# jiahansu/GPUAR

Measured on AMD Instinct MI355X. Metric: encode+decode GB/s, higher is better.
Workload: dtype u16

## Files before the change

### gpuar_amd/csrc/gpuar_kernels.hip

```cpp
#include <hip/hip_runtime.h>
#include <mutex>
#include <stdint.h>
#include <stdio.h>
#include <stdlib.h>
#include <string.h>

#include "gpuar_hip.h"

#include "lane_codec.h"
#include "crc32.h"

namespace gpuar {

__constant__ RecipTable g_recip = RecipTable();
struct MulTable {
    uint32_t m[kPacket + 64];
    constexpr MulTable() : m{} {
        const RecipTable r = RecipTable();
        for (uint32_t i = 0; i < kPacket + 64; ++i) m[i] = r.r[i < kPacket ? i : kPacket - 1u].mul;
    }
};
__device__ const MulTable g_mul = MulTable();
__constant__ DecodeConstTable g_decode = DecodeConstTable();
__device__ uint32_t g_status = 0;
// ... 19 lines not shown
        const uint32_t other = __shfl_xor(v, off);
        v = other > v ? other : v;
    }
    return __builtin_amdgcn_readfirstlane(v);
}

constexpr uint32_t kPhase = 8;
constexpr int kPrioTop = 3, kPrioCoder = 0, kPrioLow = 2;

constexpr uint32_t kRingSlots = 3;
struct alignas(16) EncodeLds {
    uint8_t tree[kTreeRows * kLanes * 2];
    uint32_t sums[kRingSlots][kPhase][kLanes];
    uint32_t bytes[2][kPhase / 4][kLanes];
};
__device__ __forceinline__ uint32_t next_slot(uint32_t slot) { return slot == kRingSlots - 1u ? 0u : slot + 1u; }

__device__ __forceinline__ size_t xcd_contiguous_group(uint32_t block, uint32_t grid) {
    const uint32_t per_xcd = grid >> 3;
    return static_cast<size_t>(block & 7u) * per_xcd + (block >> 3);
}

__device__ __forceinline__ void lds_barrier() {
    asm volatile("s_waitcnt lgkmcnt(0)\n\ts_barrier" ::: "memory");
}

__device__ __forceinline__ uint4 load16_guarded(const uint8_t *p, size_t avail) {
    if (avail >= 16) return *reinterpret_cast<const uint4 *>(p);
    uint32_t w[4] = {0, 0, 0, 0};
    for (size_t b = 0; b < avail; ++b) w[b >> 2] |= static_cast<uint32_t>(p[b]) << (8u * (b & 3u));
    return make_uint4(w[0], w[1], w[2], w[3]);
}

__device__ __forceinline__ uint32_t byte_tag(uint32_t word, uint32_t kByte) {
    uint32_t t;
    const uint32_t seven = 7u;
    if (kByte == 0) asm("v_lshlrev_b32_sdwa %0, %1, %2 dst_sel:DWORD dst_unused:UNUSED_PAD src0_sel:DWORD src1_sel:BYTE_0" : "=v"(t) : "v"(seven), "v"(word));
    if (kByte == 1) asm("v_lshlrev_b32_sdwa %0, %1, %2 dst_sel:DWORD dst_unused:UNUSED_PAD src0_sel:DWORD src1_sel:BYTE_1" : "=v"(t) : "v"(seven), "v"(word));
    if (kByte == 2) asm("v_lshlrev_b32_sdwa %0, %1, %2 dst_sel:DWORD dst_unused:UNUSED_PAD src0_sel:DWORD src1_sel:BYTE_2" : "=v"(t) : "v"(seven), "v"(word));
    if (kByte == 3) asm("v_lshlrev_b32_sdwa %0, %1, %2 dst_sel:DWORD dst_unused:UNUSED_PAD src0_sel:DWORD src1_sel:BYTE_3" : "=v"(t) : "v"(seven), "v"(word));
    return t;
}

template <bool kBatch = false>
__device__ __forceinline__ void run_top(EncodeLds &lds, const uint8_t *in, uint32_t lane, uint32_t len,
                                        uint32_t len_min, uint32_t n_phases, uint32_t whole_max = 0) {
    constexpr uint32_t kChunkPhases = 8;
    constexpr uint32_t kChunk = kChunkPhases * kPhase;
    constexpr uint32_t kPieces = kChunk / 16u;
    TopModeler<7> model;
    uint32_t k = 0, slot = 0;
    {
        const uint32_t first = len ? load16_guarded(in, len).x & 0xFFu : 0u;
        model.open(lds.tree, 2u * lane_column(lane), first);
    }
    const uint32_t full_chunks = len_min / kChunk;
    if (full_chunks) {
        const uint4 *src = reinterpret_cast<const uint4 *>(in);
        auto fetch = [&](uint32_t chunk, uint4 (&into)[kPieces]) {
#pragma unroll
            for (uint32_t t = 0; t < kPieces; ++t) {
                const uint32_t at = chunk * kChunk + 16u * t;
                if (at + 16u <= len) into[t] = src[kPieces * chunk + t];
                else if (at < len) into[t] = load16_guarded(in + at, len - at);
                else into[t] = make_uint4(0, 0, 0, 0);
            }
        };
        uint4 c[kPieces], n[kPieces], nn[kPieces];
        fetch(0, c);
        fetch(1, n);
#pragma unroll
        for (uint32_t t = 0; t < kPieces; ++t) nn[t] = make_uint4(0, 0, 0, 0);
        for (uint32_t q = 0; q < full_chunks; ++q) {
            if (q & 1u) {
                fetch(q + 1u, n);
                fetch(q + 2u, nn);
            }
            uint32_t w[kChunk / 4u + 1u];
#pragma unroll
            for (uint32_t t = 0; t < kPieces; ++t) w[4 * t] = c[t].x, w[4 * t + 1] = c[t].y, w[4 * t + 2] = c[t].z, w[4 * t + 3] = c[t].w;
            w[kChunk / 4u] = n[0].x;
#pragma unroll
            for (uint32_t ph = 0; ph < kChunkPhases; ++ph) {
                uint32_t *out = &lds.sums[slot][0][lane];
                lds.bytes[ph & 1u][0][lane] = w[2 * ph];
                lds.bytes[ph & 1u][1][lane] = w[2 * ph + 1];
#pragma unroll
                for (uint32_t j = 0; j < kPhase; ++j) {
                    const uint32_t i = ph * kPhase + j;
                    const uint32_t xn_tag = byte_tag(w[(i + 1) >> 2], (i + 1) & 3u);
                    out[j * kLanes] = model.step_tag(model.next_tag, 256u + q * kChunk + i, xn_tag);
                }
                slot = next_slot(slot);
                lds_barrier();
            }
#pragma unroll
            for (uint32_t t = 0; t < kPieces; ++t) c[t] = n[t], n[t] = nn[t];
        }
        k = kChunkPhases * full_chunks;
    }
    uint4 cur = make_uint4(0, 0, 0, 0), nxt = cur;
    if (k * kPhase < len) cur = load16_guarded(in + k * kPhase, len - k * kPhase);
    if (k * kPhase + 16u < len) nxt = load16_guarded(in + k * kPhase + 16u, len - (k * kPhase + 16u));
    if constexpr (kBatch) {
        const uint32_t whole = len / kPhase;
        for (; k < whole_max; ++k) {
            const uint32_t base = k * kPhase;
// ... 22 lines not shown
            const uint32_t own = whole * kPhase, part = len - own;
            const uint4 v = part ? load16_guarded(in + own, part) : make_uint4(0, 0, 0, 0);
            lds.bytes[k & 1u][0][lane] = v.x;
            lds.bytes[k & 1u][1][lane] = v.y;
            uint32_t *out = &lds.sums[slot][0][lane];
            uint64_t w = (static_cast<uint64_t>(v.y) << 32) | v.x;
#pragma unroll 1
            for (uint32_t j = 0; j < part; ++j) {
                const uint32_t x = static_cast<uint32_t>(w) & 0xFFu;
                w >>= 8;
                out[j * kLanes] = model.step(x, 256u + own + j, static_cast<uint32_t>(w) & 0xFFu);
            }
            slot = next_slot(slot);
            lds_barrier();
            ++k;
        }
        for (; k < n_phases + 2u; ++k) lds_barrier();
        return;
    }
    for (; k < n_phases + 2u; ++k) {
        if (k < n_phases) {
            const uint32_t base = k * kPhase;
            const bool odd = (k & 1u) != 0u;
            const uint32_t words[3] = {odd ? cur.z : cur.x, odd ? cur.w : cur.y, odd ? nxt.x : cur.z};
            if (odd) {
                cur = nxt;
                const uint32_t ahead = base + kPhase + 16u;
                if (ahead < len) nxt = load16_guarded(in + ahead, len - ahead);
                else nxt = make_uint4(0, 0, 0, 0);
            }
            uint32_t *out = &lds.sums[slot][0][lane];
            lds.bytes[k & 1u][0][lane] = words[0];
            lds.bytes[k & 1u][1][lane] = words[1];
#pragma unroll
            for (uint32_t q = 0; q < 2; ++q) {
                uint32_t w = words[q], w_next = words[q + 1];
#pragma unroll 1
                for (uint32_t b = 0; b < 4; ++b) {
                    const uint32_t i = base + 4u * q + b;
                    const uint32_t x = w & 0xFFu;
                    w = (w >> 8) | (w_next << 24);
                    w_next >>= 8;
                    if (i < len) *out = model.step(x, 256u + i, w & 0xFFu);
                    out += kLanes;
                }
            }
            slot = next_slot(slot);
        }
        lds_barrier();
    }
}

__device__ __forceinline__ void run_low(EncodeLds &lds, uint32_t lane, uint32_t len, uint32_t len_min, uint32_t n_phases) {
    LowModeler<7> model;
    model.open(lds.tree, 2u * lane_column(lane), 0u);
    lds_barrier();
    uint32_t slot = 0, k = 0;
    const uint32_t whole_phases = len_min / kPhase < n_phases ? len_min / kPhase : n_phases;
    for (; k < whole_phases; ++k) {
        const uint32_t base = k * kPhase;
        uint32_t *io = &lds.sums[slot][0][lane];
        {
            uint32_t part[kPhase], tag[kPhase];
            const uint32_t bytes[2] = {lds.bytes[k & 1u][0][lane], lds.bytes[k & 1u][1][lane]};
#pragma unroll
            for (uint32_t j = 0; j < kPhase; ++j) part[j] = io[j * kLanes], tag[j] = byte_tag(bytes[j >> 2], j & 3u);
            model.prime_tag(tag[0]);
#pragma unroll
            for (uint32_t j = 0; j < kPhase; ++j) {
                if (j + 1u < kPhase) io[j * kLanes] = model.step_tag(tag[j], 256u + base + j, tag[j + 1u], part[j]);
                else io[j * kLanes] = model.step_last_tag(tag[j], 256u + base + j, part[j]);
            }
        }
        slot = next_slot(slot);
        lds_barrier();
    }
    for (; k < n_phases; ++k) {
        const uint32_t base = k * kPhase;
        uint32_t *io = &lds.sums[slot][0][lane];
        const uint32_t bytes[2] = {lds.bytes[k & 1u][0][lane], lds.bytes[k & 1u][1][lane]};
        {
#pragma unroll 1
            for (uint32_t j = 0; j < kPhase; ++j) {
                const uint32_t i = base + j;
                if (i < len) {
                    const uint32_t t = model.tree.tag((bytes[j >> 2] >> (8u * (j & 3u))) & 0xFFu);
                    model.prime_tag(t);
                    io[j * kLanes] = model.step_last_tag(t, 256u + i, io[j * kLanes]);
                }
            }
        }
        slot = next_slot(slot);
        lds_barrier();
    }
    lds_barrier();
}

template <typename Coder>
__device__ __forceinline__ void coder_open(Coder &coder, uint8_t *dst, size_t group, uint32_t lane) {
    __builtin_amdgcn_s_setprio(kPrioCoder);
    coder.open(dst + group * (kLanes * kSlot), lane * kSlot);
    lds_barrier();
    lds_barrier();
}

template <typename Lane>
__device__ __forceinline__ void finish_lane(Lane &coder, bool live, uint32_t len, uint32_t *status) {
    if (live) {
// ... 7 lines not shown
encode_kernel(const uint8_t *__restrict__ src, size_t size, uint8_t *__restrict__ dst, uint32_t n_packets, uint32_t *__restrict__ status) {
    __shared__ EncodeLds lds;

    const size_t group = xcd_contiguous_group(blockIdx.x, gridDim.x);
    if (group * kLanes >= n_packets) return;
    const uint32_t lane = threadIdx.x & 63u;
    const uint32_t wave = __builtin_amdgcn_readfirstlane(threadIdx.x >> 6);
    const uint32_t hw = __builtin_amdgcn_s_getreg(4 | (0 << 6) | (31 << 11));
    const uint32_t simd = (hw >> 4) & 3u;
    uint32_t *hello = &lds.sums[0][0][0];
    if (lane == 0) hello[wave] = simd;
    if (threadIdx.x == 0) {
        const uint32_t xcc = __builtin_amdgcn_s_getreg(20 | (0 << 6) | (3 << 11));
        hello[4] = atomicAdd(&g_cu_ticket[((xcc & 7u) << 8) | ((hw >> 8) & 0xFFu)], 1u);
    }
    __syncthreads();
    const uint32_t seen = (1u << hello[0]) | (1u << hello[1]) | (1u << hello[2]) | (1u << hello[3]);
    const uint32_t by_simd = (simd - hello[4] - 1u) & 3u;
    const uint32_t role = __builtin_amdgcn_readfirstlane(seen == 0xFu ? by_simd : wave);
    __syncthreads();
    const size_t packet = group * kLanes + lane;
    const bool live = packet < n_packets;
    const size_t start = packet * kPacket;
    const uint32_t len = live ? static_cast<uint32_t>(size - start < kPacket ? size - start : kPacket) : 0u;
    const uint32_t len_max = wave_max(len);
    const uint32_t len_min = wave_max(~len) ^ 0xFFFFFFFFu;
    const uint32_t n_phases = (len_max + kPhase - 1) / kPhase;
    const uint8_t *in = src + (live ? start : 0);

    if (role == 0) {
        __builtin_amdgcn_s_setprio(kPrioTop);
        run_top(lds, in, lane, len, len_min, n_phases);
    } else if (role == 1) {
        __builtin_amdgcn_s_setprio(kPrioLow);
        run_low(lds, lane, len, len_min, n_phases);
    } else if (role == 3) {
        uint32_t *courier = reinterpret_cast<uint32_t *>(lds.tree + 255u * 128u);
        const uint32_t *table = reinterpret_cast<const uint32_t *>(g_recip.r);
        const uint32_t lane16 = lane & 15u;
        clock_sample(0u, group, lane, 0u);
        uint32_t carried = table[lane16];
        for (uint32_t k = 0; k < n_phases + 2u; ++k) {
            if (lane < 16u) courier[((k + 1u) & 1u) * 16u + lane16] = carried;
            const uint32_t next_phase = k < n_phases ? k : 0u;
            carried = table[next_phase * 16u + lane16];
            lds_barrier();
        }
        clock_sample(0u, group, lane, 1u);
    } else {
        CarryCoderLane coder;
        coder_open(coder, dst, group, lane);
        uint32_t slot = 0, k = 0;
        const uint32_t whole_phases = len_min / kPhase < n_phases ? len_min / kPhase : n_phases;
        for (; k < whole_phases; ++k) {
            const uint32_t *in_ring = &lds.sums[slot][0][lane];
            {
                uint32_t cums[kPhase];
#pragma unroll
                for (uint32_t j = 0; j < kPhase; ++j) cums[j] = in_ring[j * kLanes];
                Recip rc[kPhase];
                {
                    const uint4 *slot = reinterpret_cast<const uint4 *>(lds.tree + 255u * 128u + (k & 1u) * 64u);
#pragma unroll
                    for (uint32_t q = 0; q < 4; ++q) {
                        const uint4 v = slot[q];
                        rc[2 * q] = {v.x, v.y}, rc[2 * q + 1] = {v.z, v.w};
                    }
                }
                CarryCoderLane::Ahead next = coder.ahead(cums[0], rc[0]);
#pragma unroll
                for (uint32_t j = 0; j < kPhase; ++j) {
                    const CarryCoderLane::Narrowed now = coder.narrow(next);
                    if (j + 1u < kPhase) next = coder.ahead(cums[j + 1u], rc[j + 1u]);
                    coder.settle(now);
                }
            }
            slot = next_slot(slot);
            lds_barrier();
        }
        for (; k < n_phases; ++k) {
            const uint32_t base = k * kPhase;
            const uint32_t *in_ring = &lds.sums[slot][0][lane];
            {
#pragma unroll 1
                for (uint32_t j = 0; j < kPhase; ++j) {
                    const uint32_t i = base + j;
                    if (i >= len_max) break;
                    const Recip r = g_recip.r[i];
                    if (i < len) coder.step(in_ring[j * kLanes], r);
                }
            }
            slot = next_slot(slot);
            lds_barrier();
        }
        if (live) {
            bool overflowed;
            coder.finish(len, overflowed);
            if (overflowed) atomicOr(status, GPUAR_STATUS_SLOT_OVERFLOW);
        }
    }
}

__device__ __forceinline__ void batch_low(EncodeLds &lds, uint32_t lane, uint32_t len, uint32_t len_min, uint32_t n_phases, uint32_t whole_max) {
    LowModeler<7> model;
    model.open(lds.tree, 2u * lane_column(lane), 0u);
    lds_barrier();
    uint32_t slot = 0, k = 0;
    auto whole_phase = [&](uint32_t k) __attribute__((always_inline)) {
        const uint32_t base = k * kPhase;
        uint32_t *io = &lds.sums[slot][0][lane];
        uint32_t part[kPhase], tag[kPhase];
        const uint32_t bytes[2] = {lds.bytes[k & 1u][0][lane], lds.bytes[k & 1u][1][lane]};
#pragma unroll
        for (uint32_t j = 0; j < kPhase; ++j) part[j] = io[j * kLanes], tag[j] = byte_tag(bytes[j >> 2], j & 3u);
        model.prime_tag(tag[0]);
#pragma unroll
        for (uint32_t j = 0; j < kPhase; ++j) {
            if (j + 1u < kPhase) io[j * kLanes] = model.step_tag(tag[j], 256u + base + j, tag[j + 1u], part[j]);
            else io[j * kLanes] = model.step_last_tag(tag[j], 256u + base + j, part[j]);
        }
    };
    const uint32_t whole_min = len_min / kPhase;
    for (; k < whole_min; ++k) {
        whole_phase(k);
        slot = next_slot(slot);
        lds_barrier();
    }
    const uint32_t whole = len / kPhase;
// ... 1682 lines not shown
```

### gpuar_amd/csrc/lane_codec.h

```cpp
#ifndef GPUAR_LANE_CODEC_H
#define GPUAR_LANE_CODEC_H

#include <stdint.h>
#include <string.h>

#include "gpuar_hip.h"
#if defined(__HIP_DEVICE_COMPILE__) || defined(__HIPCC__)
#define GPUAR_LANE __device__ __forceinline__
#define GPUAR_CLZ32(x) static_cast<uint32_t>(__clz(static_cast<int>(x)))
#define GPUAR_CLZ32_NZ(x) static_cast<uint32_t>(__builtin_clz(x))
#define GPUAR_MULHI(a, b) __umulhi((a), (b))
#define GPUAR_MUL24(a, b) __umul24((a), (b))
#define GPUAR_AGREE_COUNT(kff, a, h, span) ([](uint32_t &k_, uint32_t a_, uint32_t h_, uint32_t &s_) { uint32_t e_; asm("v_xor_b32_sdwa %0, %3, %4 dst_sel:WORD_1 dst_unused:UNUSED_PRESERVE src0_sel:DWORD src1_sel:DWORD\n\tv_bfi_b32 %1, %3, %4, -1\n\tv_ffbh_u32 %2, %0" : "+v"(k_), "=&v"(s_), "=&v"(e_) : "v"(a_), "v"(h_)); return e_; }((kff), (a), (h), (span)))
#define GPUAR_BFM(w, off) ([](uint32_t w_, uint32_t o_) { uint32_t r_; asm("v_bfm_b32 %0, %1, %2" : "=v"(r_) : "v"(w_), "v"(o_)); return r_; }((w), (off)))
#define GPUAR_MUL24_VV(a, b) ([](uint32_t a_, uint32_t b_) { uint32_t r_; asm("v_mul_u32_u24 %0, %1, %2" : "=v"(r_) : "v"(a_), "v"(b_)); return r_; }((a), (b)))
#define GPUAR_MAD24(a, b, c) ([](uint32_t a_, uint32_t b_, uint32_t c_) { uint32_t r_; asm("v_mad_u32_u24 %0, %1, %2, %3" : "=v"(r_) : "v"(a_), "v"(b_), "v"(c_)); return r_; }((a), (b), (c)))
#define GPUAR_MAD24_VS(a, b, c) ([](uint32_t a_, uint32_t b_, uint32_t c_) { uint32_t r_; asm("v_mad_u32_u24 %0, %1, %2, %3" : "=v"(r_) : "v"(a_), "s"(b_), "v"(c_)); return r_; }((a), (b), (c)))
#define GPUAR_OR_WHERE_BIT(a, bit, b, c) ([](uint32_t a_, uint32_t b_, uint32_t c_) { uint32_t m_, r_; asm("v_bfe_i32 %0, %1, %2, 1" : "=v"(m_) : "v"(a_), "n"(bit)); asm("v_and_or_b32 %0, %1, %2, %3" : "=v"(r_) : "v"(m_), "s"(b_), "v"(c_)); return r_; }((a), (b), (c)))
#define GPUAR_XOR1_ADD(a, b) ([](uint32_t a_, uint32_t b_) { uint32_t r_; asm("v_xad_u32 %0, %1, 1, %2" : "=v"(r_) : "v"(a_), "v"(b_)); return r_; }((a), (b)))
#define GPUAR_ALIGNBIT(hi, lo, s) __builtin_amdgcn_alignbit((hi), (lo), (s))
#define GPUAR_BFE16(v, off) ([](uint32_t v_, uint32_t o_) { uint32_t r_; asm("v_bfe_u32 %0, %1, %2, 16" : "=v"(r_) : "v"(v_), "v"(o_)); return r_; }((v), (off)))
#define GPUAR_LSHL_ADD(a, s, c) ([](uint32_t a_, uint32_t s_, uint32_t c_) { uint32_t r_; asm("v_lshl_add_u32 %0, %1, %2, %3" : "=v"(r_) : "v"(a_), "v"(s_), "v"(c_)); return r_; }((a), (s), (c)))
#define GPUAR_OPAQUE_V(x) ([](uint32_t x_) { asm("" : "+v"(x_)); return x_; }((x)))
#define GPUAR_PIN_LOAD(q) asm volatile("" : : : "memory")
#define GPUAR_PIN_ORDER(x) asm volatile("" : "+v"(x) : : "memory")
#else
#define GPUAR_LANE inline
#define GPUAR_CLZ32(x) ((x) ? static_cast<uint32_t>(__builtin_clz(x)) : 32u)
#define GPUAR_CLZ32_NZ(x) static_cast<uint32_t>(__builtin_clz(x))
#define GPUAR_AGREE_COUNT(kff, a, h, span) ((span) = ~(a) | (h), static_cast<uint32_t>(__builtin_clz(((((a) ^ (h)) << 16) | 0xFFFFu))))
#define GPUAR_MULHI(a, b) static_cast<uint32_t>((static_cast<uint64_t>(a) * (b)) >> 32)
#define GPUAR_MUL24(a, b) ((a) * (b))
#define GPUAR_MUL24_VV(a, b) ((a) * (b))
#define GPUAR_BFM(w, off) (((1u << ((w) & 31u)) - 1u) << ((off) & 31u))
#define GPUAR_XOR1_ADD(a, b) ((((a) ^ 1u)) + (b))
#define GPUAR_MAD24(a, b, c) ((a) * (b) + (c))
#define GPUAR_MAD24_VS(a, b, c) ((a) * (b) + (c))
#define GPUAR_OR_WHERE_BIT(a, bit, b, c) (((((a) >> (bit)) & 1u) ? (b) : 0u) | (c))
#define GPUAR_ALIGNBIT(hi, lo, s) static_cast<uint32_t>(((static_cast<uint64_t>(hi) << 32) | (lo)) >> ((s) & 31u))
#define GPUAR_BFE16(v, off) (((v) >> ((off) & 31u)) & 0xFFFFu)
#define GPUAR_LSHL_ADD(a, s, c) (((a) << ((s) & 31u)) + (c))
#define GPUAR_PIN_ORDER(x) ((void)0)
#define GPUAR_PIN_LOAD(q) ((void)0)
#define GPUAR_OPAQUE_V(x) (x)
#endif

namespace gpuar {

constexpr uint32_t kPacket = GPUAR_PACKET_BYTES;
constexpr uint32_t kSlot = GPUAR_SLOT_BYTES;
constexpr uint32_t kHdr = GPUAR_PACKET_HEADER_BYTES;
constexpr uint32_t kLanes = 64;
constexpr uint32_t kTreeRows = 256;
constexpr uint32_t kDecodeRecords = 36;

struct Recip {
    uint32_t mul;
    uint32_t shift;
};

struct RecipTable {
    Recip r[kPacket];
    constexpr RecipTable() : r{} {
        for (uint32_t i = 0; i < kPacket; ++i) {
            const uint64_t d = 256u + i;
            uint32_t l = 8;
            while ((1ull << l) <= d) ++l;
            const uint64_t m = ((1ull << (30 + l)) + d - 1) / d;
            r[i].mul = static_cast<uint32_t>(m);
            r[i].shift = l - 2;
        }
    }
};

GPUAR_LANE uint32_t div_total(uint32_t n, Recip rc) { return GPUAR_MULHI(n, rc.mul) >> rc.shift; }


GPUAR_LANE uint32_t renorm_count(uint32_t a, uint32_t wd) {
    const uint32_t h = a + wd - 1u;
    const uint32_t d1 = (wd << 16) - 0x8000u;
    const uint32_t differ = (((a ^ h) & 0xFFFFu) << 16) | 0xFFFFu;
    const uint32_t c = GPUAR_CLZ32_NZ(d1);
    return c + ((differ << (c & 31u)) >> 31) - 1u;
}

GPUAR_LANE uint32_t bswap32(uint32_t v) { return __builtin_bswap32(v); }

struct Quad {
    uint32_t w[4];
};
// ... 35 lines not shown
    const uint32_t w[2] = {a, b};
    memcpy(at, w, 8);
#endif
}
GPUAR_LANE void store16(uint8_t *at, uint32_t v) {
#if defined(__HIP_DEVICE_COMPILE__)
    *reinterpret_cast<uint16_t *>(at) = static_cast<uint16_t>(v);
#else
    const uint16_t h = static_cast<uint16_t>(v);
    memcpy(at, &h, 2);
#endif
}

GPUAR_LANE uint32_t load32(const uint8_t *at) {
#if defined(__HIP_DEVICE_COMPILE__)
    return *reinterpret_cast<const uint32_t *>(at);
#else
    uint32_t v;
    memcpy(&v, at, 4);
    return v;
#endif
}

GPUAR_LANE void store32(uint8_t *at, uint32_t v) {
#if defined(__HIP_DEVICE_COMPILE__)
    *reinterpret_cast<uint32_t *>(at) = v;
#else
    memcpy(at, &v, 4);
#endif
}


template <uint32_t kRowShift>
struct InorderModel {
    uint8_t *table;
    uint32_t lane_bits;

    GPUAR_LANE uint32_t tag(uint32_t x) const { return x << kRowShift; }
    GPUAR_LANE uint16_t *node(uint32_t x_tag, int k) const {
        const uint32_t keep = ((0xFF00u >> k) & 0xFFu) << kRowShift;
        const uint32_t fixed = ((1u << (7 - k)) - 1u) << kRowShift;
        return reinterpret_cast<uint16_t *>(table + ((x_tag & keep) | lane_bits) + fixed);
    }
};

template <uint32_t kRowShift, int kFirst, int kDepths, int kHead, bool kTail>
struct PartialModeler {
    InorderModel<kRowShift> tree;
    uint32_t root, half0, half1;
    uint32_t halves;
    uint32_t left[kDepths];
    uint16_t *where[kDepths];

    GPUAR_LANE void open(uint8_t *table, uint32_t lane_bits, uint32_t first_symbol) {
        tree.table = table;
        tree.lane_bits = lane_bits;
#pragma unroll 1
        for (uint32_t row = 0; row < 255u; ++row) {
            const uint32_t trailing_ones = 31u - GPUAR_CLZ32((row ^ (row + 1u)));
            const int depth = 7 - static_cast<int>(trailing_ones);
            if (depth >= kFirst && depth < kFirst + kDepths)
                *reinterpret_cast<uint16_t *>(table + (row << kRowShift) + lane_bits) = static_cast<uint16_t>(1u << trailing_ones);
        }
        root = 128u;
        half0 = half1 = 64u;
        halves = 64u * 0x10001u;
        prime(first_symbol);
    }

    GPUAR_LANE void prime(uint32_t x) { prime_tag(tree.tag(x)); }
    GPUAR_LANE void prime_tag(uint32_t x_tag) {
        next_tag = x_tag;
#pragma unroll
        for (int k = 0; k < kDepths; ++k) {
            where[k] = tree.node(x_tag, kFirst + k);
            left[k] = *where[k];
        }
    }

    GPUAR_LANE static uint32_t paths_of_symbol(uint32_t x) { return GPUAR_MUL24(x, 0x10001u) + 0x10000u; }
    GPUAR_LANE static uint32_t paths_of_tag(uint32_t x_tag) { return GPUAR_MUL24(x_tag, 0x10001u) + (0x10000u << kRowShift); }

    GPUAR_LANE uint32_t step_last(uint32_t x, uint32_t total, uint32_t onto = 0) { return account<0, false>(paths_of_symbol(x), total, 0u, onto); }
    GPUAR_LANE uint32_t step_last_tag(uint32_t x_tag, uint32_t total, uint32_t onto = 0) {
        return account<static_cast<int>(kRowShift), false>(paths_of_tag(x_tag), total, 0u, onto);
    }

    GPUAR_LANE uint32_t step(uint32_t x, uint32_t total, uint32_t x_next, uint32_t onto = 0) {
        return account<0, true>(paths_of_symbol(x), total, tree.tag(x_next), onto);
    }
    GPUAR_LANE uint32_t step_tag(uint32_t x_tag, uint32_t total, uint32_t xn_tag, uint32_t onto = 0) {
        return account<static_cast<int>(kRowShift), true>(paths_of_tag(x_tag), total, xn_tag, onto);
    }

    uint32_t next_tag;

  private:
    template <int kShift, bool kAhead>
    GPUAR_LANE uint32_t account(uint32_t z, uint32_t total, uint32_t xn, uint32_t onto) {
        uint32_t acc = onto;
        if (kTail) acc = GPUAR_OR_WHERE_BIT(z, kShift + 24, total << 16, onto);
        if (kHead == 1 || kHead == 2) {
            const uint32_t pick0 = (z >> (kShift + 7)) & 0x10001u;
            acc = GPUAR_MAD24(root, pick0, acc);
            root = GPUAR_XOR1_ADD(pick0, root) & 0xFFFFu;
        }
        if (kHead == 3) {
            const uint32_t pick1 = (z >> (kShift + 6)) & 0x10001u;
            const uint32_t where1 = (z >> (kShift + 3)) & 16u;
            acc = GPUAR_MAD24(GPUAR_BFE16(halves, where1), pick1, acc);
            halves = GPUAR_LSHL_ADD(~pick1 & 1u, where1, halves);
        }
        if (kHead == 2) {
            static_assert(kHead != 2 || (kShift == 0 && kAhead), "depths 0 and 1 in registers: symbol-based step() only");
            const uint32_t x = z & 0xFFu;
            const bool upper_half = x >= 128u;
            const uint32_t pick1 = (z >> 6) & 0x10001u;
            acc = GPUAR_MAD24(upper_half ? half1 : half0, pick1, acc);
            const uint32_t quarter = x >> 6;
            half0 += quarter == 0u ? 1u : 0u;
            half1 += quarter == 2u ? 1u : 0u;
        }
#pragma unroll
        for (int k = 0; k < kDepths; ++k) {
            const uint32_t pick = (z >> (kShift + 7 - (kFirst + k))) & 0x10001u;
            const uint32_t l = left[k];
            acc = GPUAR_MAD24(l, pick, acc);
            *where[k] = static_cast<uint16_t>(GPUAR_XOR1_ADD(pick, l));
            if (kAhead) {
                where[k] = tree.node(xn, kFirst + k);
                left[k] = *where[k];
            }
        }
        if (kAhead) next_tag = xn;
        return acc;
    }
};

#ifndef GPUAR_TOP_DEPTHS
#define GPUAR_TOP_DEPTHS 4
#endif
#if defined(GPUAR_TOP_D1_REGS)
template <uint32_t kRowShift>
using TopModeler = PartialModeler<kRowShift, 2, GPUAR_TOP_DEPTHS - 1, 3, false>;
#else
template <uint32_t kRowShift>
using TopModeler = PartialModeler<kRowShift, 1, GPUAR_TOP_DEPTHS, 0, false>;
#endif
template <uint32_t kRowShift>
using LowModeler = PartialModeler<kRowShift, 1 + GPUAR_TOP_DEPTHS, 7 - GPUAR_TOP_DEPTHS, 1, true>;
template <uint32_t kRowShift>
using DeepestModeler = PartialModeler<kRowShift, 7, 1, 1, true>;

struct CoderLane {
    uint32_t lo;
    uint32_t range;
    uint32_t pending;
    uint32_t acc;
    uint32_t n;
    uint32_t at;
    uint32_t last;
    uint32_t kff;
    uint8_t *base;
    uint32_t body_off;

    GPUAR_LANE void open(uint8_t *uniform_base, uint32_t slot_offset) {
        lo = 0;
        range = 0x10000u;
        pending = 0;
        acc = 0;
        n = 0;
        kff = 0xFFFFu;
        base = uniform_base;
        body_off = slot_offset + kHdr;
        at = body_off;
        last = slot_offset + kSlot - 4u;
    }

    GPUAR_LANE void put(uint32_t bits, uint32_t count) {
        const uint32_t total = n + count;
        const uint32_t left_aligned = bits << ((32u - count) & 31u);
        const uint32_t word = GPUAR_ALIGNBIT(acc, left_aligned, n);
#if defined(__HIP_DEVICE_COMPILE__)
        acc = (acc << (count & 31u)) | bits;
        {
            const unsigned long long full = __builtin_amdgcn_ballot_w64(total >= 32u);
            unsigned long long saved;
            uint32_t t_addr, t_word, t_mask;
            asm volatile(
                "s_and_saveexec_b64 %[sx], %[m]\n\t"
                "v_min_u32 %[ta], %[at], %[last]\n\t"
                "v_perm_b32 %[tw], 0, %[word], %[sel]\n\t"
                "global_store_dword %[ta], %[tw], %[base]\n\t"
                "v_add_u32 %[at], 4, %[at]\n\t"
                "v_bfm_b32 %[tm], %[total], 0\n\t"
                "v_and_b32 %[acc], %[bits], %[tm]\n\t"
                "s_or_b64 exec, exec, %[sx]"
                : [at] "+v"(at), [acc] "+v"(acc), [ta] "=&v"(t_addr), [tw] "=&v"(t_word), [tm] "=&v"(t_mask), [sx] "=&s"(saved)
                : [m] "s"(full), [last] "v"(last), [word] "v"(word), [sel] "s"(0x00010203u), [base] "s"(base), [total] "v"(total), [bits] "v"(bits)
                : "scc", "memory");
        }
#else
        acc = (acc << (count & 31u)) | bits;
// ... 72 lines not shown
    uint32_t range;
    uint32_t held;
    uint32_t cache;
    uint32_t nff;
    uint32_t at;
    uint32_t last;
    uint32_t kff;
    uint8_t *base;
    uint32_t body_off;

    GPUAR_LANE void open(uint8_t *uniform_base, uint32_t slot_offset) {
        wl = 0;
        wh = 0;
        range = 0x10000u;
#if defined(__HIP_DEVICE_COMPILE__)
        held = 16u;
#else
        held = 0;
#endif
        cache = 0;
        nff = 0;
        kff = 0xFFFFu;
        base = uniform_base;
        body_off = slot_offset + kHdr;
        at = slot_offset;
        last = slot_offset + kSlot - 4u;
    }

    GPUAR_LANE void store_clamped(uint32_t word) {
        store32(base + (at < last ? at : last), bswap32(word));
        at += 4u;
    }

    GPUAR_LANE uint32_t take_top(uint32_t &over) {
        const uint32_t s = held - 16u;
        const uint32_t word = GPUAR_ALIGNBIT(wh, wl, s);
        over = wh >> s;
        wl &= GPUAR_BFM(s, 0u);
        wh = 0;
        held -= 32u;
        return word;
    }

    GPUAR_LANE void leave(uint32_t word, uint32_t over) {
        if (word != 0xFFFFFFFFu || over) {
            store_clamped(cache + over);
            for (; nff; --nff) store_clamped(over ? 0u : 0xFFFFFFFFu);
            cache = word;
        } else {
            ++nff;
        }
    }

#if defined(__HIP_DEVICE_COMPILE__)
    GPUAR_LANE void shift_and_store(uint32_t n, unsigned long long full) {
        unsigned long long saved, rare, undecided;
        uint32_t over, sent, t_addr, t_swapped;
        {
            const uint64_t w = ((static_cast<uint64_t>(wh) << 32) | wl) << n;
            wl = static_cast<uint32_t>(w), wh = static_cast<uint32_t>(w >> 32);
        }
        asm volatile(
            "s_and_saveexec_b64 %[sx], %[m]\n\t"
            "v_lshrrev_b32 %[over], %[held], %[wh]\n\t"
            "v_add_u32 %[sent], %[cache], %[over]\n\t"
            "v_alignbit_b32 %[cache], %[wh], %[wl], %[held]\n\t"
            "v_cmp_ge_u32 %[rare], %[cache], %[key]\n\t"
            "v_min_u32 %[ta], %[at], %[last]\n\t"
            "v_perm_b32 %[tw], 0, %[sent], %[sel]\n\t"
            "global_store_dword %[ta], %[tw], %[base]\n\t"
            "v_bfe_u32 %[wl], %[wl], 0, %[held]\n\t"
            "v_mov_b32 %[wh], 0\n\t"
            "v_add_u32 %[at], 4, %[at]\n\t"
            "v_add_u32 %[held], -32, %[held]\n\t"
            "s_or_b64 exec, exec, %[sx]\n\t"
            "s_cmp_eq_u64 %[rare], 0\n\t"
            "s_cbranch_scc1 .Lgpuar_common_%=\n\t"
            "s_mov_b64 %[sx], exec\n\t"
            "s_mov_b64 exec, %[rare]\n\t"
            "v_cmp_eq_u32 vcc, -1, %[cache]\n\t"
            "v_cmp_eq_u32 %[und], 0, %[over]\n\t"
            "v_cndmask_b32 %[tw], 0, -1, %[und]\n\t"
            "s_and_b64 %[und], %[und], vcc\n\t"
            "s_and_b64 exec, %[rare], %[und]\n\t"
            "v_add_u32 %[at], -4, %[at]\n\t"
            "v_mov_b32 %[cache], %[sent]\n\t"
            "v_add_u32 %[nff], 1, %[nff]\n\t"
            "s_andn2_b64 exec, %[rare], %[und]\n\t"
            ".Lgpuar_fill_%=:\n\t"
            "v_cmp_ne_u32 vcc, 0, %[nff]\n\t"
            "s_and_b64 exec, exec, vcc\n\t"
            "s_cbranch_execz .Lgpuar_filled_%=\n\t"
            "v_min_u32 %[ta], %[at], %[last]\n\t"
            "global_store_dword %[ta], %[tw], %[base]\n\t"
            "v_add_u32 %[at], 4, %[at]\n\t"
            "v_add_u32 %[nff], -1, %[nff]\n\t"
            "s_branch .Lgpuar_fill_%=\n\t"
            ".Lgpuar_filled_%=:\n\t"
            "s_mov_b64 exec, %[rare]\n\t"
            "v_cmp_eq_u32 vcc, 0, %[nff]\n\t"
            "v_cndmask_b32 %[key], 0, -1, vcc\n\t"
            "s_mov_b64 exec, %[sx]\n\t"
            ".Lgpuar_common_%=:"
            : [wl] "+v"(wl), [wh] "+v"(wh), [at] "+v"(at), [held] "+v"(held), [cache] "+v"(cache), [nff] "+v"(nff), [key] "+v"(key),
              [over] "=&v"(over), [sent] "=&v"(sent), [ta] "=&v"(t_addr), [tw] "=&v"(t_swapped),
              [sx] "=&s"(saved), [rare] "=&s"(rare), [und] "=&s"(undecided)
            : [m] "s"(full), [last] "v"(last), [sel] "s"(0x00010203u), [base] "s"(base)
            : "memory", "vcc", "scc");
    }
#endif

#if defined(__HIP_DEVICE_COMPILE__)
    GPUAR_LANE unsigned long long settled_mask(uint32_t n, uint32_t wd) {
        unsigned long long full;
        asm volatile("v_add_u32 %[held], %[held], %[n]\n\t"
                     "v_cmp_le_u32 %[m], 48, %[held]\n\t"
                     "v_lshlrev_b32 %[rng], %[n], %[wd]"
                     : [held] "+v"(held), [m] "=&s"(full), [rng] "=v"(range)
                     : [n] "v"(n), [wd] "v"(wd));
        return full;
    }
#endif

    struct Ahead {
        uint32_t dn, wd;
    };
    struct Narrowed {
        uint32_t n;
        unsigned long long full;
    };
    GPUAR_LANE Ahead ahead(uint32_t cums, Recip rc) const {
#if defined(__HIP_DEVICE_COMPILE__)
        uint32_t up, dn;
        asm volatile("v_mul_u32_u24_sdwa %[up], %[c], %[r] dst_sel:DWORD dst_unused:UNUSED_PAD src0_sel:WORD_1 src1_sel:DWORD\n\t"
                     "v_mul_u32_u24_sdwa %[dn], %[c], %[r] dst_sel:DWORD dst_unused:UNUSED_PAD src0_sel:WORD_0 src1_sel:DWORD\n\t"
                     "v_mul_hi_u32 %[up], %[up], %[m]\n\t"
                     "v_mul_hi_u32 %[dn], %[dn], %[m]\n\t"
                     "v_lshrrev_b32 %[up], %[s], %[up]\n\t"
                     "v_lshrrev_b32 %[dn], %[s], %[dn]\n\t"
                     "v_sub_u32 %[up], %[up], %[dn]"
                     : [up] "=&v"(up), [dn] "=&v"(dn)
                     : [c] "v"(cums), [r] "v"(range), [m] "v"(rc.mul), [s] "v"(rc.shift));
        return {dn, up};
#else
        const uint32_t up = div_total(GPUAR_MUL24(cums >> 16, range), rc);
        const uint32_t dn = div_total(GPUAR_MUL24(cums & 0xFFFFu, range), rc);
        return {dn, up - dn};
#endif
    }
    GPUAR_LANE Narrowed narrow(Ahead a) {
        const uint32_t dn = a.dn, wd = a.wd;
#if defined(__HIP_DEVICE_COMPILE__)
        uint32_t h, t2, c, t, n;
        asm("v_add_co_u32 %[wl], vcc, %[wl], %[dn]\n\t"
            "v_addc_co_u32 %[wh], vcc, 0, %[wh], vcc\n\t"
            "v_add3_u32 %[h], %[wl], %[wd], -1\n\t"
            "v_lshl_add_u32 %[t2], %[wd], 16, %[km]\n\t"
            "v_xor_b32_sdwa %[kff], %[wl], %[h] dst_sel:WORD_1 dst_unused:UNUSED_PRESERVE src0_sel:WORD_0 src1_sel:WORD_0\n\t"
            "v_ffbh_u32 %[c], %[t2]\n\t"
            "v_lshlrev_b32 %[t], %[c], %[kff]\n\t"
            "v_lshrrev_b32 %[t], 31, %[t]\n\t"
            "v_add3_u32 %[n], %[c], %[t], -1"
            : [wl] "+v"(wl), [wh] "+v"(wh), [kff] "+v"(kff), [h] "=&v"(h), [t2] "=&v"(t2), [c] "=&v"(c), [t] "=&v"(t), [n] "=&v"(n)
            : [dn] "v"(dn), [wd] "v"(wd), [km] "s"(0xFFFF8000u)
            : "vcc");
        const unsigned long long full = settled_mask(n, wd);
        return {n, full};
#else
        const uint64_t sum = ((static_cast<uint64_t>(wh) << 32) | wl) + dn;
        wl = static_cast<uint32_t>(sum), wh = static_cast<uint32_t>(sum >> 32);
        const uint32_t n = renorm_count(wl & 0xFFFFu, wd);
        range = wd << n;
        held += n;
// ... 352 lines not shown
```

Before: 202.1.

## Hand-schedule full coder phase in one asm block and unroll tree init

Replaces the per-symbol ahead/narrow/settle loop in the carry coder with a single inline-asm block that handles all eight symbols of a phase, pinning the 64-bit window to fixed registers. The intent is to remove compiler-inserted moves and waits between symbols. It also adds a packed 16-bit multiply-add head variant for the low modeler, fully unrolls tree-table initialisation for non-batch paths, and toggles the courier slot offset with an opaque XOR instead of computing it from k. Hard-coding v110/v111 risks register clobbers or conflicts and raises register pressure.

```diff
diff --git a/gpuar_amd/csrc/gpuar_kernels.hip b/gpuar_amd/csrc/gpuar_kernels.hip
--- a/gpuar_amd/csrc/gpuar_kernels.hip
+++ b/gpuar_amd/csrc/gpuar_kernels.hip
@@ -95,7 +95,7 @@
     uint32_t k = 0, slot = 0;
     {
         const uint32_t first = len ? load16_guarded(in, len).x & 0xFFu : 0u;
-        model.open(lds.tree, 2u * lane_column(lane), first);
+        model.open<!kBatch>(lds.tree, 2u * lane_column(lane), first);
     }
     const uint32_t full_chunks = len_min / kChunk;
     if (full_chunks) {
@@ -224,8 +224,8 @@
 }
 
 __device__ __forceinline__ void run_low(EncodeLds &lds, uint32_t lane, uint32_t len, uint32_t len_min, uint32_t n_phases) {
-    LowModeler<7> model;
-    model.open(lds.tree, 2u * lane_column(lane), 0u);
+    PhaseLowModeler<7> model;
+    model.open<true>(lds.tree, 2u * lane_column(lane), 0u);
     lds_barrier();
     uint32_t slot = 0, k = 0;
     const uint32_t whole_phases = len_min / kPhase < n_phases ? len_min / kPhase : n_phases;
@@ -339,6 +339,7 @@
         coder_open(coder, dst, group, lane);
         uint32_t slot = 0, k = 0;
         const uint32_t whole_phases = len_min / kPhase < n_phases ? len_min / kPhase : n_phases;
+        uint32_t pairs_at = GPUAR_OPAQUE_V(0u);
         for (; k < whole_phases; ++k) {
             const uint32_t *in_ring = &lds.sums[slot][0][lane];
             {
@@ -347,20 +348,15 @@
                 for (uint32_t j = 0; j < kPhase; ++j) cums[j] = in_ring[j * kLanes];
                 Recip rc[kPhase];
                 {
-                    const uint4 *slot = reinterpret_cast<const uint4 *>(lds.tree + 255u * 128u + (k & 1u) * 64u);
+                    const uint4 *slot = reinterpret_cast<const uint4 *>(lds.tree + 255u * 128u + pairs_at);
+                    pairs_at ^= 64u;
 #pragma unroll
                     for (uint32_t q = 0; q < 4; ++q) {
                         const uint4 v = slot[q];
                         rc[2 * q] = {v.x, v.y}, rc[2 * q + 1] = {v.z, v.w};
                     }
                 }
-                CarryCoderLane::Ahead next = coder.ahead(cums[0], rc[0]);
-#pragma unroll
-                for (uint32_t j = 0; j < kPhase; ++j) {
-                    const CarryCoderLane::Narrowed now = coder.narrow(next);
-                    if (j + 1u < kPhase) next = coder.ahead(cums[j + 1u], rc[j + 1u]);
-                    coder.settle(now);
-                }
+                coder.phase(cums, rc);
             }
             slot = next_slot(slot);
             lds_barrier();
diff --git a/gpuar_amd/csrc/lane_codec.h b/gpuar_amd/csrc/lane_codec.h
--- a/gpuar_amd/csrc/lane_codec.h
+++ b/gpuar_amd/csrc/lane_codec.h
@@ -15,6 +15,7 @@
 #define GPUAR_BFM(w, off) ([](uint32_t w_, uint32_t o_) { uint32_t r_; asm("v_bfm_b32 %0, %1, %2" : "=v"(r_) : "v"(w_), "v"(o_)); return r_; }((w), (off)))
 #define GPUAR_MUL24_VV(a, b) ([](uint32_t a_, uint32_t b_) { uint32_t r_; asm("v_mul_u32_u24 %0, %1, %2" : "=v"(r_) : "v"(a_), "v"(b_)); return r_; }((a), (b)))
 #define GPUAR_MAD24(a, b, c) ([](uint32_t a_, uint32_t b_, uint32_t c_) { uint32_t r_; asm("v_mad_u32_u24 %0, %1, %2, %3" : "=v"(r_) : "v"(a_), "v"(b_), "v"(c_)); return r_; }((a), (b), (c)))
+#define GPUAR_MAD16_PAIR(a, b, c) ([](uint32_t a_, uint32_t b_, uint32_t c_) { uint32_t r_; asm("v_pk_mad_u16 %0, %1, %2, %3 op_sel_hi:[0,1,1]" : "=v"(r_) : "v"(a_), "v"(b_), "v"(c_)); return r_; }((a), (b), (c)))
 #define GPUAR_MAD24_VS(a, b, c) ([](uint32_t a_, uint32_t b_, uint32_t c_) { uint32_t r_; asm("v_mad_u32_u24 %0, %1, %2, %3" : "=v"(r_) : "v"(a_), "s"(b_), "v"(c_)); return r_; }((a), (b), (c)))
 #define GPUAR_OR_WHERE_BIT(a, bit, b, c) ([](uint32_t a_, uint32_t b_, uint32_t c_) { uint32_t m_, r_; asm("v_bfe_i32 %0, %1, %2, 1" : "=v"(m_) : "v"(a_), "n"(bit)); asm("v_and_or_b32 %0, %1, %2, %3" : "=v"(r_) : "v"(m_), "s"(b_), "v"(c_)); return r_; }((a), (b), (c)))
 #define GPUAR_XOR1_ADD(a, b) ([](uint32_t a_, uint32_t b_) { uint32_t r_; asm("v_xad_u32 %0, %1, 1, %2" : "=v"(r_) : "v"(a_), "v"(b_)); return r_; }((a), (b)))
@@ -36,6 +37,7 @@
 #define GPUAR_XOR1_ADD(a, b) ((((a) ^ 1u)) + (b))
 #define GPUAR_MAD24(a, b, c) ((a) * (b) + (c))
 #define GPUAR_MAD24_VS(a, b, c) ((a) * (b) + (c))
+#define GPUAR_MAD16_PAIR(a, b, c) (((a) & 0xFFFFu) * (b) + (c))
 #define GPUAR_OR_WHERE_BIT(a, bit, b, c) (((((a) >> (bit)) & 1u) ? (b) : 0u) | (c))
 #define GPUAR_ALIGNBIT(hi, lo, s) static_cast<uint32_t>(((static_cast<uint64_t>(hi) << 32) | (lo)) >> ((s) & 31u))
 #define GPUAR_BFE16(v, off) (((v) >> ((off) & 31u)) & 0xFFFFu)
@@ -177,20 +179,28 @@
     uint32_t left[kDepths];
     uint16_t *where[kDepths];
 
+    template <bool kStraight = false>
     GPUAR_LANE void open(uint8_t *table, uint32_t lane_bits, uint32_t first_symbol) {
         tree.table = table;
         tree.lane_bits = lane_bits;
+        if (kStraight) {
+#pragma unroll
+            for (uint32_t row = 0; row < 255u; ++row) init_row(table, lane_bits, row);
+        } else {
 #pragma unroll 1
-        for (uint32_t row = 0; row < 255u; ++row) {
-            const uint32_t trailing_ones = 31u - GPUAR_CLZ32((row ^ (row + 1u)));
-            const int depth = 7 - static_cast<int>(trailing_ones);
-            if (depth >= kFirst && depth < kFirst + kDepths)
-                *reinterpret_cast<uint16_t *>(table + (row << kRowShift) + lane_bits) = static_cast<uint16_t>(1u << trailing_ones);
+            for (uint32_t row = 0; row < 255u; ++row) init_row(table, lane_bits, row);
         }
         root = 128u;
         half0 = half1 = 64u;
         halves = 64u * 0x10001u;
         prime(first_symbol);
+    }
+
+    GPUAR_LANE static void init_row(uint8_t *table, uint32_t lane_bits, uint32_t row) {
+        const uint32_t trailing_ones = 31u - GPUAR_CLZ32((row ^ (row + 1u)));
+        const int depth = 7 - static_cast<int>(trailing_ones);
+        if (depth >= kFirst && depth < kFirst + kDepths)
+            *reinterpret_cast<uint16_t *>(table + (row << kRowShift) + lane_bits) = static_cast<uint16_t>(1u << trailing_ones);
     }
 
     GPUAR_LANE void prime(uint32_t x) { prime_tag(tree.tag(x)); }
@@ -229,6 +239,11 @@
             const uint32_t pick0 = (z >> (kShift + 7)) & 0x10001u;
             acc = GPUAR_MAD24(root, pick0, acc);
             root = GPUAR_XOR1_ADD(pick0, root) & 0xFFFFu;
+        }
+        if (kHead == 4) {
+            const uint32_t pick0 = (z >> (kShift + 7)) & 0x10001u;
+            acc = GPUAR_MAD16_PAIR(root, pick0, acc);
+            root = GPUAR_XOR1_ADD(pick0, root);
         }
         if (kHead == 3) {
             const uint32_t pick1 = (z >> (kShift + 6)) & 0x10001u;
@@ -274,6 +289,8 @@
 #endif
 template <uint32_t kRowShift>
 using LowModeler = PartialModeler<kRowShift, 1 + GPUAR_TOP_DEPTHS, 7 - GPUAR_TOP_DEPTHS, 1, true>;
+template <uint32_t kRowShift>
+using PhaseLowModeler = PartialModeler<kRowShift, 1 + GPUAR_TOP_DEPTHS, 7 - GPUAR_TOP_DEPTHS, 4, true>;
 template <uint32_t kRowShift>
 using DeepestModeler = PartialModeler<kRowShift, 7, 1, 1, true>;
 
@@ -452,6 +469,48 @@
         }
     }
 
+#define GPUAR_CODER_STORE_TEXT(ID) \
+    "s_and_saveexec_b64 %[sx], %[m]\n\t"                                                                                                \
+    "v_lshrrev_b32 %[over], %[held], %[wh]\n\t"                                                                                         \
+    "v_add_u32 %[sent], %[cache], %[over]\n\t"                      \
+    "v_alignbit_b32 %[cache], %[wh], %[wl], %[held]\n\t"                       \
+    "v_cmp_ge_u32 %[rare], %[cache], %[key]\n\t"                                          \
+    "v_min_u32 %[ta], %[at], %[last]\n\t"                                                                                               \
+    "v_perm_b32 %[tw], 0, %[sent], %[sel]\n\t"                                                                                          \
+    "global_store_dword %[ta], %[tw], %[base]\n\t"                                                                                      \
+    "v_bfe_u32 %[wl], %[wl], 0, %[held]\n\t"                                    \
+    "v_mov_b32 %[wh], 0\n\t"                                                                                                            \
+    "v_add_u32 %[at], 4, %[at]\n\t"                                                                                                     \
+    "v_add_u32 %[held], -32, %[held]\n\t"                                                                                               \
+    "s_or_b64 exec, exec, %[sx]\n\t"                                                                                                    \
+    "s_cmp_eq_u64 %[rare], 0\n\t"                                                                                                       \
+    "s_cbranch_scc1 .Lgpuar_common_" ID "\n\t"                                                                                          \
+    "s_mov_b64 %[sx], exec\n\t"                                                                                                         \
+    "s_mov_b64 exec, %[rare]\n\t"                                                                                                       \
+    "v_cmp_eq_u32 vcc, -1, %[cache]\n\t"                                                                                                \
+    "v_cmp_eq_u32 %[und], 0, %[over]\n\t"                                                                                               \
+    "v_cndmask_b32 %[tw], 0, -1, %[und]\n\t"                             \
+    "s_and_b64 %[und], %[und], vcc\n\t"                                                                                                 \
+    "s_and_b64 exec, %[rare], %[und]\n\t"                                                                             \
+    "v_add_u32 %[at], -4, %[at]\n\t"                                                                                                    \
+    "v_mov_b32 %[cache], %[sent]\n\t"                                                                                                   \
+    "v_add_u32 %[nff], 1, %[nff]\n\t"                                                                                                   \
+    "s_andn2_b64 exec, %[rare], %[und]\n\t"                                                                             \
+    ".Lgpuar_fill_" ID ":\n\t"                                                                                                          \
+    "v_cmp_ne_u32 vcc, 0, %[nff]\n\t"                                                                                                   \
+    "s_and_b64 exec, exec, vcc\n\t"                                                                                                     \
+    "s_cbranch_execz .Lgpuar_filled_" ID "\n\t"                                                                                         \
+    "v_min_u32 %[ta], %[at], %[last]\n\t"                                                                                               \
+    "global_store_dword %[ta], %[tw], %[base]\n\t"                                                                                      \
+    "v_add_u32 %[at], 4, %[at]\n\t"                                                                                                     \
+    "v_add_u32 %[nff], -1, %[nff]\n\t"                                                                                                  \
+    "s_branch .Lgpuar_fill_" ID "\n\t"                                                                                                  \
+    ".Lgpuar_filled_" ID ":\n\t"                                                                                                        \
+    "s_mov_b64 exec, %[rare]\n\t"                                                                                                       \
+    "v_cmp_eq_u32 vcc, 0, %[nff]\n\t"                                                                                                   \
+    "v_cndmask_b32 %[key], 0, -1, vcc\n\t"                                                                                              \
+    "s_mov_b64 exec, %[sx]\n\t"                                                                                                         \
+    ".Lgpuar_common_" ID ":"                                                                                                           
 #if defined(__HIP_DEVICE_COMPILE__)
     GPUAR_LANE void shift_and_store(uint32_t n, unsigned long long full) {
         unsigned long long saved, rare, undecided;
@@ -461,47 +520,7 @@
             wl = static_cast<uint32_t>(w), wh = static_cast<uint32_t>(w >> 32);
         }
         asm volatile(
-            "s_and_saveexec_b64 %[sx], %[m]\n\t"
-            "v_lshrrev_b32 %[over], %[held], %[wh]\n\t"
-            "v_add_u32 %[sent], %[cache], %[over]\n\t"
-            "v_alignbit_b32 %[cache], %[wh], %[wl], %[held]\n\t"
-            "v_cmp_ge_u32 %[rare], %[cache], %[key]\n\t"
-            "v_min_u32 %[ta], %[at], %[last]\n\t"
-            "v_perm_b32 %[tw], 0, %[sent], %[sel]\n\t"
-            "global_store_dword %[ta], %[tw], %[base]\n\t"
-            "v_bfe_u32 %[wl], %[wl], 0, %[held]\n\t"
-            "v_mov_b32 %[wh], 0\n\t"
-            "v_add_u32 %[at], 4, %[at]\n\t"
-            "v_add_u32 %[held], -32, %[held]\n\t"
-            "s_or_b64 exec, exec, %[sx]\n\t"
-            "s_cmp_eq_u64 %[rare], 0\n\t"
-            "s_cbranch_scc1 .Lgpuar_common_%=\n\t"
-            "s_mov_b64 %[sx], exec\n\t"
-            "s_mov_b64 exec, %[rare]\n\t"
-            "v_cmp_eq_u32 vcc, -1, %[cache]\n\t"
-            "v_cmp_eq_u32 %[und], 0, %[over]\n\t"
-            "v_cndmask_b32 %[tw], 0, -1, %[und]\n\t"
-            "s_and_b64 %[und], %[und], vcc\n\t"
-            "s_and_b64 exec, %[rare], %[und]\n\t"
-            "v_add_u32 %[at], -4, %[at]\n\t"
-            "v_mov_b32 %[cache], %[sent]\n\t"
-            "v_add_u32 %[nff], 1, %[nff]\n\t"
-            "s_andn2_b64 exec, %[rare], %[und]\n\t"
-            ".Lgpuar_fill_%=:\n\t"
-            "v_cmp_ne_u32 vcc, 0, %[nff]\n\t"
-            "s_and_b64 exec, exec, vcc\n\t"
-            "s_cbranch_execz .Lgpuar_filled_%=\n\t"
-            "v_min_u32 %[ta], %[at], %[last]\n\t"
-            "global_store_dword %[ta], %[tw], %[base]\n\t"
-            "v_add_u32 %[at], 4, %[at]\n\t"
-            "v_add_u32 %[nff], -1, %[nff]\n\t"
-            "s_branch .Lgpuar_fill_%=\n\t"
-            ".Lgpuar_filled_%=:\n\t"
-            "s_mov_b64 exec, %[rare]\n\t"
-            "v_cmp_eq_u32 vcc, 0, %[nff]\n\t"
-            "v_cndmask_b32 %[key], 0, -1, vcc\n\t"
-            "s_mov_b64 exec, %[sx]\n\t"
-            ".Lgpuar_common_%=:"
+            GPUAR_CODER_STORE_TEXT("%=")
             : [wl] "+v"(wl), [wh] "+v"(wh), [at] "+v"(at), [held] "+v"(held), [cache] "+v"(cache), [nff] "+v"(nff), [key] "+v"(key),
               [over] "=&v"(over), [sent] "=&v"(sent), [ta] "=&v"(t_addr), [tw] "=&v"(t_swapped),
               [sx] "=&s"(saved), [rare] "=&s"(rare), [und] "=&s"(undecided)
@@ -519,6 +538,63 @@
                      : [held] "+v"(held), [m] "=&s"(full), [rng] "=v"(range)
                      : [n] "v"(n), [wd] "v"(wd));
         return full;
+    }
+#endif
+
+#if defined(__HIP_DEVICE_COMPILE__)
+#define GPUAR_CODER_WINDOW "v[110:111]"
+#define GPUAR_CODER_AHEAD_TEXT(J)                                                                                              \
+    "v_mul_u32_u24_sdwa %[up], %[c" J "], %[rng] dst_sel:DWORD dst_unused:UNUSED_PAD src0_sel:WORD_1 src1_sel:DWORD\n\t"        \
+    "v_mul_u32_u24_sdwa %[dn], %[c" J "], %[rng] dst_sel:DWORD dst_unused:UNUSED_PAD src0_sel:WORD_0 src1_sel:DWORD\n\t"        \
+    "v_mul_hi_u32 %[up], %[up], %[m" J "]\n\t"                                                                                   \
+    "v_mul_hi_u32 %[dn], %[dn], %[m" J "]\n\t"                                                                                   \
+    "v_lshrrev_b32 %[up], %[s" J "], %[up]\n\t"                                                                                  \
+    "v_lshrrev_b32 %[dn], %[s" J "], %[dn]\n\t"                                                                                  \
+    "v_sub_u32 %[up], %[up], %[dn]\n\t"
+#define GPUAR_CODER_NARROW_TEXT                                                                                                \
+    "v_add_co_u32 %[wl], vcc, %[wl], %[dn]\n\t"                                                                                  \
+    "v_addc_co_u32 %[wh], vcc, 0, %[wh], vcc\n\t"                                                                                \
+    "v_add3_u32 %[h], %[wl], %[up], -1\n\t"                                                                                      \
+    "v_lshl_add_u32 %[t2], %[up], 16, %[km]\n\t"                                                                                 \
+    "v_xor_b32_sdwa %[kff], %[wl], %[h] dst_sel:WORD_1 dst_unused:UNUSED_PRESERVE src0_sel:WORD_0 src1_sel:WORD_0\n\t"           \
+    "v_ffbh_u32 %[c], %[t2]\n\t"                                                                                                 \
+    "v_lshlrev_b32 %[t], %[c], %[kff]\n\t"                                                                                       \
+    "v_lshrrev_b32 %[t], 31, %[t]\n\t"                                                                                           \
+    "v_add3_u32 %[n], %[c], %[t], -1\n\t"                                                                                        \
+    "v_add_u32 %[held], %[held], %[n]\n\t"                                                                                       \
+    "v_cmp_le_u32 %[m], 48, %[held]\n\t"                                                                                         \
+    "v_lshlrev_b32 %[rng], %[n], %[up]\n\t"                                                                                      \
+    "v_lshlrev_b64 " GPUAR_CODER_WINDOW ", %[n], " GPUAR_CODER_WINDOW "\n\t"
+#define GPUAR_CODER_SYMBOL_TEXT(J, NEXT) GPUAR_CODER_NARROW_TEXT GPUAR_CODER_AHEAD_TEXT(NEXT) GPUAR_CODER_STORE_TEXT("%=_" J) "\n\t"
+    GPUAR_LANE void phase(const uint32_t (&cums)[8], const Recip (&rc)[8]) {
+        register uint32_t lo asm("v110") = wl;
+        register uint32_t hi asm("v111") = wh;
+        unsigned long long full, saved, rare, undecided;
+        uint32_t up, dn, h, t2, c, t, n, over, sent, t_addr, t_swapped;
+        asm volatile(
+            GPUAR_CODER_AHEAD_TEXT("0")
+            GPUAR_CODER_SYMBOL_TEXT("0", "1") GPUAR_CODER_SYMBOL_TEXT("1", "2") GPUAR_CODER_SYMBOL_TEXT("2", "3")
+            GPUAR_CODER_SYMBOL_TEXT("3", "4") GPUAR_CODER_SYMBOL_TEXT("4", "5") GPUAR_CODER_SYMBOL_TEXT("5", "6")
+            GPUAR_CODER_SYMBOL_TEXT("6", "7")
+            GPUAR_CODER_NARROW_TEXT GPUAR_CODER_STORE_TEXT("%=_7")
+            : [wl] "+v"(lo), [wh] "+v"(hi), [rng] "+v"(range), [at] "+v"(at), [held] "+v"(held), [cache] "+v"(cache), [nff] "+v"(nff),
+              [key] "+v"(key), [kff] "+v"(kff),
+              [up] "=&v"(up), [dn] "=&v"(dn), [h] "=&v"(h), [t2] "=&v"(t2), [c] "=&v"(c), [t] "=&v"(t), [n] "=&v"(n),
+              [over] "=&v"(over), [sent] "=&v"(sent), [ta] "=&v"(t_addr), [tw] "=&v"(t_swapped),
+              [m] "=&s"(full), [sx] "=&s"(saved), [rare] "=&s"(rare), [und] "=&s"(undecided)
+            : [c0] "v"(cums[0]), [c1] "v"(cums[1]), [c2] "v"(cums[2]), [c3] "v"(cums[3]), [c4] "v"(cums[4]), [c5] "v"(cums[5]),
+              [c6] "v"(cums[6]), [c7] "v"(cums[7]),
+              [m0] "v"(rc[0].mul), [m1] "v"(rc[1].mul), [m2] "v"(rc[2].mul), [m3] "v"(rc[3].mul), [m4] "v"(rc[4].mul),
+              [m5] "v"(rc[5].mul), [m6] "v"(rc[6].mul), [m7] "v"(rc[7].mul),
+              [s0] "v"(rc[0].shift), [s1] "v"(rc[1].shift), [s2] "v"(rc[2].shift), [s3] "v"(rc[3].shift), [s4] "v"(rc[4].shift),
+              [s5] "v"(rc[5].shift), [s6] "v"(rc[6].shift), [s7] "v"(rc[7].shift),
+              [km] "s"(0xFFFF8000u), [last] "v"(last), [sel] "s"(0x00010203u), [base] "s"(base)
+            : "memory", "vcc", "scc");
+        wl = lo, wh = hi;
+    }
+#else
+    GPUAR_LANE void phase(const uint32_t (&cums)[8], const Recip (&rc)[8]) {
+        for (uint32_t j = 0; j < 8u; ++j) settle(narrow(ahead(cums[j], rc[j])));
     }
 #endif
 
```

New measurement: 203.7 (median of 6 runs). About the same (+0.8%).
